# MariaPdg/thesis-fmri-reconstruction

Measured on NVIDIA B200. Metric: stage1_vaegan_train_samples_per_sec_64x64, higher is better.
Workload: dtype bf16

## Files before the change

thesis_fmri_reconstruction_b200/csrc/api.cu:

```cuda
#include <cstdarg>
#include <cstdio>
#include <cstring>
#include <cstdlib>
#include <algorithm>

#include "../../include/fmri_b200.h"
#include "simt_kernels.cuh"
#include "tc_kernels.cuh"
#include "hconv_kernels.cuh"
#include "hwgrad_kernels.cuh"
#include "cto3_kernels.cuh"
#include "mmd_kernels.cuh"
#include "eval_kernels.cuh"

using namespace fmri;

static thread_local char g_err[512] = "";
static int fail(int code, const char* fmt, ...) {
    va_list ap;
    va_start(ap, fmt);
    vsnprintf(g_err, sizeof(g_err), fmt, ap);
    va_end(ap);
    return code;
}
// ... 39 lines not shown
    }
    void* p = nullptr;
    return cudaMallocAsync(&p, bytes, st) == cudaSuccess ? p : nullptr;
}
#define SCRATCH(ptr, type, count, st)                                                                        \
    type* ptr = reinterpret_cast<type*>(scratch_alloc(sizeof(type) * (size_t)(count), st));                  \
    if (!ptr) return fail(FMRI_ERR_CUDA, "scratch allocation of %zu bytes", sizeof(type) * (size_t)(count))
template <typename T>
static int ordered_add(const T* part, int nparts, long long n, T* dst, cudaStream_t st) {
    ordered_add_kernel<T><<<grid1d(n, 256), 256, 0, st>>>(part, nparts, n, dst);
    LAUNCH_OK();
    return 0;
}

extern "C" int fmri_tensor_path_available(void) {
    int dev = 0, major = 0;
    if (cudaGetDevice(&dev) != cudaSuccess) {
        cudaGetLastError();
        return 0;
    }
    if (cudaDeviceGetAttribute(&major, cudaDevAttrComputeCapabilityMajor, dev) != cudaSuccess) {
        cudaGetLastError();
        return 0;
    }
    return major == 10 ? 1 : 0;
}

typedef CUresult (*EncodeTiledFn)(CUtensorMap*, CUtensorMapDataType, cuuint32_t, void*, const cuuint64_t*,
                                  const cuuint64_t*, const cuuint32_t*, const cuuint32_t*, CUtensorMapInterleave,
                                  CUtensorMapSwizzle, CUtensorMapL2promotion, CUtensorMapFloatOOBfill);
static EncodeTiledFn encode_fn() {
    static EncodeTiledFn fn = [] {
        void* p = nullptr;
        cudaDriverEntryPointQueryResult q;
        if (cudaGetDriverEntryPoint("cuTensorMapEncodeTiled", &p, cudaEnableDefault, &q) != cudaSuccess) p = nullptr;
        return reinterpret_cast<EncodeTiledFn>(p);
    }();
    return fn;
}
static int make_map(CUtensorMap* m, const void* base, int rank, const long long* dims, const long long* strides_el,
                    const int* box, int inner_bytes) {
    EncodeTiledFn fn = encode_fn();
    if (!fn) return fail(FMRI_ERR_CUDA, "cuTensorMapEncodeTiled entry point not found");
    cuuint64_t gd[4], gs[3];
    cuuint32_t bx[4], es[4];
    for (int i = 0; i < rank; ++i) {
        gd[i] = (cuuint64_t)dims[i];
        bx[i] = (cuuint32_t)box[i];
        es[i] = 1;
    }
    for (int i = 0; i + 1 < rank; ++i) gs[i] = (cuuint64_t)strides_el[i] * 2;
    const CUtensorMapSwizzle sw = inner_bytes == 128 ? CU_TENSOR_MAP_SWIZZLE_128B
                                 : inner_bytes == 64 ? CU_TENSOR_MAP_SWIZZLE_64B
                                                     : CU_TENSOR_MAP_SWIZZLE_32B;
    CUresult r = fn(m, CU_TENSOR_MAP_DATA_TYPE_BFLOAT16, (cuuint32_t)rank, const_cast<void*>(base), gd, gs, bx, es,
                    CU_TENSOR_MAP_INTERLEAVE_NONE, sw, CU_TENSOR_MAP_L2_PROMOTION_L2_256B,
                    CU_TENSOR_MAP_FLOAT_OOB_FILL_NONE);
    if (r != CUDA_SUCCESS)
        return fail(FMRI_ERR_CUDA,
                    "cuTensorMapEncodeTiled failed (%d): rank %d dims %lld %lld %lld %lld box %d %d %d %d stride0 %lld",
                    (int)r, rank, dims[0], dims[1], rank > 2 ? dims[2] : 0, rank > 3 ? dims[3] : 0, box[0], box[1],
                    rank > 2 ? box[2] : 0, rank > 3 ? box[3] : 0, strides_el[0]);
    return 0;
}
static int make_act_map(CUtensorMap* m, const void* base, int C, int X, int Y, int N, long long sx, long long sy,
                        long long sn, int box_c, int bw, int bh, int bn) {
    const long long dims[4] = {C, std::max(X, 1), std::max(Y, 1), N};
    const long long st[3] = {sx, sy, sn};
    const int box[4] = {box_c, bw, bh, bn};
    return make_map(m, base, 4, dims, st, box, box_c * 2);
}

template <int BN, int KCH, int STAGES, int MT>
static int launch_ig(const IgParams& p, int classes, cudaStream_t st) {
    using L = IgSmem<BN, KCH, STAGES, MT>;
    static bool attr_done = false;
    if (!attr_done) {
        CUDA_OK(cudaFuncSetAttribute(igemm_kernel<BN, KCH, STAGES, MT>, cudaFuncAttributeMaxDynamicSharedMemorySize,
                                     L::TOTAL));
        attr_done = true;
    }
    dim3 grid(cdiv((long long)p.tiles_x * p.tiles_y * p.tiles_n, MT), p.n_tiles * p.splits, classes);
    igemm_kernel<BN, KCH, STAGES, MT><<<grid, 192, L::TOTAL, st>>>(p);
    LAUNCH_OK();
    return 0;
}
template <int BN, int KCH, int STAGES, int MT, int EXTRA, bool YR = false>
static int launch_ig_persistent_x(const IgParams& p, int classes, cudaStream_t st) {
    using L = IgSmem<BN, KCH, STAGES, MT, YR, EXTRA, true>;
    static bool attr_done = false;
    if (!attr_done) {
        CUDA_OK(cudaFuncSetAttribute(igemm_persistent_kernel<BN, KCH, STAGES, MT, EXTRA, YR>,
                                     cudaFuncAttributeMaxDynamicSharedMemorySize, L::TOTAL));
        attr_done = true;
    }
    const long long m_groups = cdiv((long long)p.tiles_x * p.tiles_y * p.tiles_n, MT);
    const long long tiles = m_groups * p.n_tiles * classes;
    static int occ = 0;
    if (!occ) {
        CUDA_OK(cudaOccupancyMaxActiveBlocksPerMultiprocessor(&occ, igemm_persistent_kernel<BN, KCH, STAGES, MT, EXTRA, YR>,
                                                              IGP_THREADS, L::TOTAL));
        occ = std::max(1, occ);
    }
    const int per_sm = std::max(1, std::min<int>(std::min(2, 512 / (2 * MT * BN)), occ));
    const int grid = (int)std::min<long long>(tiles, 148LL * per_sm);
    igemm_persistent_kernel<BN, KCH, STAGES, MT, EXTRA, YR><<<grid, IGP_THREADS, L::TOTAL, st>>>(p, classes);
// ... 686 lines not shown
}

extern "C" int fmri_conv_wgrad(const fmri_conv_desc* d, const void* x, const void* dy, float* dw, int accumulate,
                               void* ws, size_t ws_bytes, void* stream) {
    int rc = check_conv(d);
    if (rc) return rc;
    int OH, OW;
    fmri_conv_out_hw(d, &OH, &OW);
    if (d->dtype == FMRI_BF16) {
        const size_t need = fmri_conv_wgrad_workspace(d);
        if (!ws || ws_bytes < need) return fail(FMRI_ERR_WORKSPACE, "conv wgrad workspace %zu < %zu", ws_bytes, need);
        if (d->stride != 2) return fail(FMRI_ERR_UNSUPPORTED, "stride-1 conv wgrad on the tensor path");
        CUDA_OK(cudaMemsetAsync(ws, 0, need, S(stream)));
        float* wsf = reinterpret_cast<float*>(ws);
        int Cd, Cs;
        if (!d->transposed) {
            Cd = d->Cout; Cs = d->Cin;
            rc = run_wgrad_tc(dy, d->N, OH, OW, Cd, x, d->H, d->W, Cs, 2, 25, wsf, S(stream));
        } else {
            Cd = d->Cin; Cs = d->Cout;
            rc = run_wgrad_tc(x, d->N, d->H, d->W, Cd, dy, OH, OW, Cs, 2, 25, wsf, S(stream));
        }
        if (rc) return rc;
        const long long n = 25LL * Cd * Cs;
        scatter4_kernel<float, float><<<grid1d(n, 256), 256, 0, S(stream)>>>(wsf, dw, 1, 25, Cd, Cs, 0, 1, 25LL * Cs,
                                                                            25, accumulate);
        LAUNCH_OK();
        return 0;
    }
    DirectWgradParams p;
    memset(&p, 0, sizeof(p));
    p.N = d->N;
    p.stride = d->stride;
    p.accumulate = accumulate;
    const float *A, *B;
    if (!d->transposed) {
        A = reinterpret_cast<const float*>(dy); p.PH = OH; p.PW = OW; p.Ca = d->Cout;
        B = reinterpret_cast<const float*>(x); p.BH = d->H; p.BW = d->W; p.Cb = d->Cin;
    } else {
        A = reinterpret_cast<const float*>(x); p.PH = d->H; p.PW = d->W; p.Ca = d->Cin;
        B = reinterpret_cast<const float*>(dy); p.BH = OH; p.BW = OW; p.Cb = d->Cout;
    }
    p.a_sn = (long long)p.PH * p.PW * p.Ca; p.a_sy = (long long)p.PW * p.Ca; p.a_sx = p.Ca; p.a_sc = 1;
    p.b_sn = (long long)p.BH * p.BW * p.Cb; p.b_sy = (long long)p.BW * p.Cb; p.b_sx = p.Cb; p.b_sc = 1;
    p.w_sa = 25LL * p.Cb;
    p.w_sb = 25;
    direct_wgrad_kernel<float, float><<<25 * p.Ca * p.Cb, 128, 0, S(stream)>>>(A, B, dw, p);
    LAUNCH_OK();
    return 0;
}

static const size_t HC_WS_PACK = 65536;
extern "C" size_t fmri_edge_workspace(const fmri_edge_desc* d) {
    return std::max(sizeof(float) * 75 * (size_t)d->C, HC_WS_PACK + (size_t)d->N * d->H * d->W * 16);
}

static bool hc_build(HcParams& p, HcPackSpec& spec, int N, int H, int W, int chunks, int stride, int OH, int OW, int BN,
                     bool flip) {
    memset(&p, 0, sizeof(p));
    memset(&spec, 0, sizeof(spec));
    p.N = N; p.H = H; p.W = W; p.chunks = chunks; p.OH = OH; p.OW = OW;
    const int hx = stride == 1 ? 4 : 2;
    if (stride == 1) {
        p.num_planes = 1;
        p.pl_ys[0] = p.pl_xs[0] = 1;
        p.pl_yoff[0] = p.pl_xoff[0] = -2;
    } else {
        p.num_planes = 4;
        for (int ph = 0; ph < 2; ++ph)
            for (int pw = 0; pw < 2; ++pw) {
                const int pl = ph * 2 + pw;
                p.pl_ys[pl] = p.pl_xs[pl] = 2;
                p.pl_yoff[pl] = ph - 2;
                p.pl_xoff[pl] = pw - 2;
            }
    }
    p.PW = OW + hx;
    if (p.PW > 200) return false;
    const int max_off = hx * p.PW + hx;
    const int nsteps = chunks >= 2 ? 25 * (chunks / 2) : 13;
    if (nsteps > HC_MAX_STEPS) return false;
    p.num_steps = nsteps;
    bool found = false;
    for (int pass = 0; pass < 2 && !found; ++pass) {
        const int mt_max = std::min(5, (pass == 0 ? 128 : 256) / BN);
        const size_t smem_cap = pass == 0 ? 110 * 1024 : 227 * 1024;
        double best = 0.0;
        for (int tht = std::min(OH, (mt_max * 128) / p.PW); tht >= 1; --tht) {
            HcParams q = p;
            q.THt = tht;
            q.tiles_y = cdiv(OH, tht);
            q.MT = cdiv((long long)tht * q.PW, 128);
            q.PH = tht + hx;
            q.slab_rows = (q.PH * q.PW + 7) / 8 * 8 + (chunks > 1 ? 2 : 0);
            const long long overshoot = ((long long)q.MT * 128 + max_off + 1 - q.slab_rows) * 16;
            if (overshoot > 0 && overshoot > hc_b_bytes(q, BN)) continue;
            if ((size_t)hc_smem_bytes(q, BN) > smem_cap) continue;
            const double eff = (double)OH * OW / ((double)q.tiles_y * q.MT * 128);
            if (eff > best + 1e-9) { best = eff; p = q; found = true; }
        }
    }
    if (!found) return false;
    int woff[25];
    for (int kh = 0; kh < 5; ++kh)
        for (int kw = 0; kw < 5; ++kw) {
            int plane = 0, dyr = kh, dxr = kw;
            if (stride == 2) {
// ... 101 lines not shown
    memset(&p, 0, sizeof(p));
    __nv_bfloat16* wt = reinterpret_cast<__nv_bfloat16*>(ws);
    c3_pack_weights_kernel<<<cdiv(C3_NB * C, 256), 256, 0, st>>>(w, wt, s_co, s_c, flip, C);
    LAUNCH_OK();
    if (make_act_map(&p.mapX, X, C, H * W, 1, N, C, (long long)H * W * C, (long long)H * W * C, C, 128, 1, 1)) return 1;
    {
        const long long dims[2] = {C, C3_NB};
        const long long stv[1] = {C};
        const int box[2] = {C, C3_NB};
        if (make_map(&p.mapW, wt, 2, dims, stv, box, C * 2)) return 1;
    }
    p.N = N; p.H = H; p.out = img; p.bias = bias; p.act = act;
    static bool attr_done = false;
    if (!attr_done) {
        CUDA_OK(cudaFuncSetAttribute(cto3_kernel, cudaFuncAttributeMaxDynamicSharedMemorySize, C3_SMEM));
        attr_done = true;
    }
    cto3_kernel<<<std::min(N, 148), C3_THREADS, C3_SMEM, st>>>(p);
    LAUNCH_OK();
    return 0;
}

static int hconv_c_to_3(const void* X, int N, int H, int W, int C, const float* w, long long s_co, long long s_c, int flip,
                        const float* bias, int act, float* img, void* ws, cudaStream_t st) {
    if (C != 32 && C != 64) return 1;
    {
        const int rc = cto3_run(X, N, H, W, C, w, s_co, s_c, flip, bias, act, img, ws, st);
        if (rc <= 0) return rc;
    }
    HcParams p;
    HcPackSpec spec;
    if (!hc_build(p, spec, N, H, W, C / 8, 1, H, W, 16, flip != 0)) return 1;
    p.X = reinterpret_cast<const __nv_bfloat16*>(X);
    p.epi = 0; p.out = img; p.bias = bias; p.act = act; p.n_out = 3;
    return hc_run(p, spec, 16, w, 3, C, s_co, s_c, ws, st);
}

static int hconv_3_to_c(const float* i0, const float* i1, const float* i2, int nps, int N, int H, int W, int C, int stride,
                        const float* w, long long s_c, long long s_ci, int flip, const float* bias, int act, void* y,
                        void* ws, cudaStream_t st) {
    if (C != 32 && C != 64) return 1;
    const int OH = (H - 1) / stride + 1, OW = (W - 1) / stride + 1;
    HcParams p;
    HcPackSpec spec;
    if (!hc_build(p, spec, N, H, W, 1, stride, OH, OW, C, flip != 0)) return 1;
    __nv_bfloat16* img8 = reinterpret_cast<__nv_bfloat16*>(reinterpret_cast<uint8_t*>(ws) + HC_WS_PACK);
    img8_pack_kernel<<<grid1d((long long)N * H * W, 256), 256, 0, st>>>(i0, i1, i2, nps, N, (long long)H * W, img8);
    LAUNCH_OK();
    p.X = img8;
    p.epi = 1; p.out = y; p.bias = bias; p.act = act; p.n_out = C;
    return hc_run(p, spec, C, w, C, 3, s_c, s_ci, ws, st);
}

static int g_hw_variant = -1;
static int hwgrad_run(const void* T, const float* i0, const float* i1, const float* i2, int nps, int N, int PH, int PW, int C,
                      float* dwk, float* dbias, int flip, void* ws, cudaStream_t st, int plane = -1, int IH = 0, int IW = 0) {
    if (g_hw_variant < 0) {
        const char* e = getenv("FMRI_HWGRAD");
        g_hw_variant = e ? atoi(e) : 0;
    }
    if (g_hw_variant == 2) return 1;
    if (C != 32 && C != 64) return 1;
    HwParams p;
    memset(&p, 0, sizeof(p));
    p.N = N; p.PH = PH; p.PW = PW; p.C = C;
    p.PWp = (PW + 4 + 15) / 16 * 16;
    if (p.PWp > 128) return 1;
    static int bh_cap = 0;
    if (!bh_cap) {
        const char* e = getenv("FMRI_HW_BH");
        bh_cap = e ? std::max(1, atoi(e)) : 2;
    }
    p.bh = std::max(1, std::min(std::min(PH, bh_cap), 256 / p.PWp));
    p.tiles_y = cdiv(PH, p.bh);
    p.slab_rows = ((p.bh + 4) * p.PWp + 16 + 7) / 8 * 8;
    p.d_chunk = (p.bh * p.PWp * 128 + 1023) / 1024 * 1024;
    p.stages = 2;
    if (hw_smem_bytes(p) > 227 * 1024) return 1;
    while (p.stages < HW_MAX_STAGES) {
        ++p.stages;
        if (hw_smem_bytes(p) > 110 * 1024) { --p.stages; break; }
    }
    const long long dims[4] = {C, PW, PH, N};
    const long long strides[3] = {C, (long long)PW * C, (long long)PH * PW * C};
    const int box[4] = {64, p.PWp, p.bh, 1};
    if (make_map(&p.mapT, T, 4, dims, strides, box, 128)) return 1;
    __nv_bfloat16* img8 = reinterpret_cast<__nv_bfloat16*>(reinterpret_cast<uint8_t*>(ws) + HC_WS_PACK);
    p.kh0 = 0; p.nkh = 5;
    if (plane < 0) {
        img8_pack_kernel<<<grid1d((long long)N * PH * PW, 256), 256, 0, st>>>(i0, i1, i2, nps, N, (long long)PH * PW, img8);
    } else {
        p.plane = 1; p.ph = plane >> 1; p.pw = plane & 1;
        p.kh0 = 1; p.nkh = p.ph ? 2 : 3;
        img8_plane_pack_kernel<<<grid1d((long long)N * PH * PW, 256), 256, 0, st>>>(i0, i1, i2, nps, N, IH, IW, PH, PW, p.ph,
                                                                                   p.pw, img8);
    }
    LAUNCH_OK();
    p.img8 = img8;
    p.dwk = dwk; p.dbias = dbias; p.flip = flip; p.desc_variant = g_hw_variant;
    const int smem = hw_smem_bytes(p);
    static int attr_smem = 0;
    if (smem > attr_smem) {
        CUDA_OK(cudaFuncSetAttribute(hwgrad_kernel, cudaFuncAttributeMaxDynamicSharedMemorySize, smem));
        attr_smem = smem;
    }
    const int total = N * p.tiles_y;
    const int nb = std::min(total, 148 * (smem <= 110 * 1024 ? 2 : 1));
    const long long nw = 75LL * C;
    SCRATCH(part, float, (long long)nb * (nw + C), st);
    CUDA_OK(cudaMemsetAsync(part, 0, sizeof(float) * (size_t)nb * (nw + C), st));
    p.dwk = part;
    p.dbias = dbias ? part + nb * nw : nullptr;
    hwgrad_kernel<<<nb, HW_THREADS, smem, st>>>(p);
    LAUNCH_OK();
    int rc = ordered_add(part, nb, nw, dwk, st);
    if (!rc && dbias) rc = ordered_add(part + nb * nw, nb, C, dbias, st);
    CUDA_OK(cudaFreeAsync(part, st));
    return rc;
}

static int check_edge(const fmri_edge_desc* d, const void* ws, size_t ws_bytes) {
    if (!d || (d->C != 32 && d->C != 64)) return fail(FMRI_ERR_UNSUPPORTED, "edge conv supports C in {32,64}");
    if (d->stride != 1 && d->stride != 2) return fail(FMRI_ERR_ARG, "edge stride");
    if (!ws || ws_bytes < fmri_edge_workspace(d)) return fail(FMRI_ERR_WORKSPACE, "edge workspace too small");
    return 0;
}
static int pack_edge_in(const fmri_edge_desc* d, const float* w, float* wk, cudaStream_t st) {
    permute4_kernel<float, float><<<grid1d(75LL * d->C, 256), 256, 0, st>>>(w, wk, 1, 3, 25, d->C, 0, 25, 1, 75, 0);
    LAUNCH_OK();
    return 0;
}
static int pack_edge_out(const fmri_edge_desc* d, const float* w, float* wk, int flip, cudaStream_t st) {
    permute4_kernel<float, float><<<grid1d(75LL * d->C, 256), 256, 0, st>>>(
        flip ? w + 24 : w, wk, 1, 3, 25, d->C, 0, 25LL * d->C, flip ? -1 : 1, 25, 0);
    LAUNCH_OK();
    return 0;
}
template <int C>
static int edge_in_fprop_t(const fmri_edge_desc* d, const float* i0, const float* i1, const float* i2, int nps,
                           const float* wk, const float* bias, int act, void* y, int OH, int OW, cudaStream_t st) {
    const long long pix = (long long)d->N * OH * OW;
    if (d->dtype == FMRI_BF16)
        edge3_to_c_kernel<C, __nv_bfloat16><<<cdiv(pix, 128), 128, 0, st>>>(
            i0, i1, i2, nps, wk, bias, reinterpret_cast<__nv_bfloat16*>(y), d->N, d->H, d->W, OH, OW, d->stride, act);
    else
        edge3_to_c_kernel<C, float><<<cdiv(pix, 128), 128, 0, st>>>(i0, i1, i2, nps, wk, bias,
                                                                   reinterpret_cast<float*>(y), d->N, d->H, d->W, OH,
                                                                   OW, d->stride, act);
    LAUNCH_OK();
    return 0;
}
extern "C" int fmri_edge_in_fprop(const fmri_edge_desc* d, const float* img0, const float* img1, const float* img2,
                                  int n_per_src, const float* w, const float* bias, int act, void* y, void* ws,
                                  size_t ws_bytes, void* stream) {
    int rc = check_edge(d, ws, ws_bytes);
    if (rc) return rc;
    if (!img1) img1 = img0;
    if (!img2) img2 = img0;
    if (d->dtype == FMRI_BF16 && fmri_tensor_path_available()) {
        rc = hconv_3_to_c(img0, img1, img2, n_per_src, d->N, d->H, d->W, d->C, d->stride, w, 75, 25, 0, bias, act, y, ws,
                          S(stream));
        if (rc <= 0) return rc;
    }
    float* wk = reinterpret_cast<float*>(ws);
    rc = pack_edge_in(d, w, wk, S(stream));
    if (rc) return rc;
    const int OH = (d->H - 1) / d->stride + 1, OW = (d->W - 1) / d->stride + 1;
// ... 24 lines not shown
    }
    float* wk = reinterpret_cast<float*>(ws);
    rc = pack_edge_in(d, w, wk, S(stream));
    if (rc) return rc;
    const int flip = d->stride == 1 ? 1 : 0;
    return d->C == 32 ? edge_to3_t<32>(d->dtype, dy, wk, nullptr, dimg, d->N, OH, OW, d->H, d->W, d->stride, flip, 0,
                                       S(stream))
                      : edge_to3_t<64>(d->dtype, dy, wk, nullptr, dimg, d->N, OH, OW, d->H, d->W, d->stride, flip, 0,
                                       S(stream));
}
template <int C>
static int edge_wgrad_t(int dtype, const void* T, const float* i0, const float* i1, const float* i2, int nps,
                        float* dwk, float* dbias, int N, int PH, int PW, int IH, int IW, int stride, int sg,
                        cudaStream_t st) {
    if (PW <= 128 && (PW - 1) * stride + 5 <= 144) {
        const long long lines = (long long)N * PH;
        const int rpb = (int)std::max<long long>(1, (lines + 148 * 3 - 1) / (148 * 3));
        const int blocks = cdiv(lines, rpb);
        if (dtype == FMRI_BF16)
            edge_wgrad_rows_kernel<C, __nv_bfloat16><<<blocks, 256, 0, st>>>(
                reinterpret_cast<const __nv_bfloat16*>(T), i0, i1, i2, nps, dwk, dbias, N, PH, PW, IH, IW, stride, sg, rpb);
        else
            edge_wgrad_rows_kernel<C, float><<<blocks, 256, 0, st>>>(reinterpret_cast<const float*>(T), i0, i1, i2, nps,
                                                                    dwk, dbias, N, PH, PW, IH, IW, stride, sg, rpb);
        LAUNCH_OK();
        return 0;
    }
    if (dbias) return fail(FMRI_ERR_UNSUPPORTED, "edge wgrad: fused bias gradient needs rows of <= 128 pixels");
    const long long pix = (long long)N * PH * PW;
    int ppb = (int)std::max<long long>(64, ((pix + 148 * 4 - 1) / (148 * 4) + 7) / 8 * 8);
    const int blocks = cdiv(pix, ppb);
    if (dtype == FMRI_BF16)
        edge_wgrad_kernel<C, __nv_bfloat16><<<blocks, 256, 0, st>>>(reinterpret_cast<const __nv_bfloat16*>(T), i0, i1,
                                                                    i2, nps, dwk, N, PH, PW, IH, IW, stride, sg, ppb);
    else
        edge_wgrad_kernel<C, float><<<blocks, 256, 0, st>>>(reinterpret_cast<const float*>(T), i0, i1, i2, nps, dwk, N,
                                                            PH, PW, IH, IW, stride, sg, ppb);
    LAUNCH_OK();
    return 0;
}
extern "C" int fmri_edge_in_wgrad(const fmri_edge_desc* d, const float* img0, const float* img1, const float* img2,
                                  int n_per_src, const void* dy, float* dw, float* dbias, int accumulate, void* ws,
                                  size_t ws_bytes, void* stream) {
    int rc = check_edge(d, ws, ws_bytes);
    if (rc) return rc;
    float* dwk = reinterpret_cast<float*>(ws);
    CUDA_OK(cudaMemsetAsync(dwk, 0, sizeof(float) * 75 * (size_t)d->C, S(stream)));
    const int OH = (d->H - 1) / d->stride + 1, OW = (d->W - 1) / d->stride + 1;
    if (!img1) img1 = img0;
    if (!img2) img2 = img0;
    if (dbias && !accumulate) CUDA_OK(cudaMemsetAsync(dbias, 0, sizeof(float) * d->C, S(stream)));
    rc = 1;
    if (d->dtype == FMRI_BF16 && d->stride == 1 && fmri_tensor_path_available())
        rc = hwgrad_run(dy, img0, img1, img2, n_per_src, d->N, d->H, d->W, d->C, dwk, dbias, 0, ws, S(stream));
    else if (d->dtype == FMRI_BF16 && d->stride == 2 && !dbias && fmri_tensor_path_available()) {
        for (int plane = 0; plane < 4; ++plane) {
            rc = hwgrad_run(dy, img0, img1, img2, n_per_src, d->N, OH, OW, d->C, dwk, nullptr, 0, ws, S(stream), plane, d->H, d->W);
            if (rc) break;
        }
        if (rc == 1) CUDA_OK(cudaMemsetAsync(dwk, 0, sizeof(float) * 75 * (size_t)d->C, S(stream)));
    }
    if (rc == 1)
        rc = d->C == 32 ? edge_wgrad_t<32>(d->dtype, dy, img0, img1, img2, n_per_src, dwk, dbias, d->N, OH, OW, d->H, d->W,
                                           d->stride, 1, S(stream))
                        : edge_wgrad_t<64>(d->dtype, dy, img0, img1, img2, n_per_src, dwk, dbias, d->N, OH, OW, d->H, d->W,
                                           d->stride, 1, S(stream));
    if (rc) return rc;
    scatter4_kernel<float, float><<<grid1d(75LL * d->C, 256), 256, 0, S(stream)>>>(dwk, dw, 1, 3, 25, d->C, 0, 25, 1,
                                                                                  75, accumulate);
    LAUNCH_OK();
    return 0;
}
extern "C" int fmri_edge_out_fprop(const fmri_edge_desc* d, const void* x, const float* w, const float* bias, int act,
                                   float* img, void* ws, size_t ws_bytes, void* stream) {
    int rc = check_edge(d, ws, ws_bytes);
    if (rc) return rc;
    if (d->stride != 1) return fail(FMRI_ERR_UNSUPPORTED, "edge out conv is stride 1");
    if (d->dtype == FMRI_BF16 && fmri_tensor_path_available()) {
        rc = hconv_c_to_3(x, d->N, d->H, d->W, d->C, w, 25LL * d->C, 25, 0, bias, act, img, ws, S(stream));
        if (rc <= 0) return rc;
    }
    float* wk = reinterpret_cast<float*>(ws);
    rc = pack_edge_out(d, w, wk, 0, S(stream));
    if (rc) return rc;
    return d->C == 32
               ? edge_to3_t<32>(d->dtype, x, wk, bias, img, d->N, d->H, d->W, d->H, d->W, 1, 0, act, S(stream))
               : edge_to3_t<64>(d->dtype, x, wk, bias, img, d->N, d->H, d->W, d->H, d->W, 1, 0, act, S(stream));
}
extern "C" int fmri_edge_out_dgrad(const fmri_edge_desc* d, const float* dimg, const float* w, void* dx, void* ws,
                                   size_t ws_bytes, void* stream) {
    int rc = check_edge(d, ws, ws_bytes);
    if (rc) return rc;
    if (d->stride != 1) return fail(FMRI_ERR_UNSUPPORTED, "edge out conv is stride 1");
    if (d->dtype == FMRI_BF16 && fmri_tensor_path_available()) {
        rc = hconv_3_to_c(dimg, dimg, dimg, d->N, d->N, d->H, d->W, d->C, 1, w, 25, 25LL * d->C, 1, nullptr, 0, dx, ws,
                          S(stream));
        if (rc <= 0) return rc;
    }
    float* wk = reinterpret_cast<float*>(ws);
    rc = pack_edge_out(d, w, wk, 1, S(stream));
    if (rc) return rc;
    fmri_edge_desc e = *d;
    return e.C == 32 ? edge_in_fprop_t<32>(&e, dimg, dimg, dimg, d->N, wk, nullptr, 0, dx, d->H, d->W, S(stream))
                     : edge_in_fprop_t<64>(&e, dimg, dimg, dimg, d->N, wk, nullptr, 0, dx, d->H, d->W, S(stream));
}
extern "C" int fmri_edge_out_wgrad(const fmri_edge_desc* d, const void* x, const float* dimg, float* dw,
                                   int accumulate, void* ws, size_t ws_bytes, void* stream) {
    int rc = check_edge(d, ws, ws_bytes);
    if (rc) return rc;
    if (d->stride != 1) return fail(FMRI_ERR_UNSUPPORTED, "edge out conv is stride 1");
    float* dwk = reinterpret_cast<float*>(ws);
    CUDA_OK(cudaMemsetAsync(dwk, 0, sizeof(float) * 75 * (size_t)d->C, S(stream)));
    rc = 1;
    if (d->dtype == FMRI_BF16 && fmri_tensor_path_available())
        rc = hwgrad_run(x, dimg, dimg, dimg, d->N, d->N, d->H, d->W, d->C, dwk, nullptr, 1, ws, S(stream));
    if (rc == 1)
        rc = d->C == 32 ? edge_wgrad_t<32>(d->dtype, x, dimg, dimg, dimg, d->N, dwk, nullptr, d->N, d->H, d->W, d->H, d->W,
                                           1, -1, S(stream))
                        : edge_wgrad_t<64>(d->dtype, x, dimg, dimg, dimg, d->N, dwk, nullptr, d->N, d->H, d->W, d->H, d->W,
                                           1, -1, S(stream));
    if (rc) return rc;
    scatter4_kernel<float, float><<<grid1d(75LL * d->C, 256), 256, 0, S(stream)>>>(dwk, dw, 1, 3, 25, d->C, 0,
                                                                                  25LL * d->C, 1, 25, accumulate);
    LAUNCH_OK();
    return 0;
}

static int transpose_any(const void* src, int sdt, void* dst, int ddt, int N, int R, int Cc, int accumulate, cudaStream_t st);
extern "C" int fmri_linear_pack_weights(const fmri_linear_desc* d, const float* w, void* wp, int ldw, void* wpt,
                                        int ldwt, void* stream) {
    if (!d || d->M < 0 || d->N <= 0 || d->K <= 0) return fail(FMRI_ERR_ARG, "bad linear descriptor");
    if (wp) {
        if (ldw < d->K) return fail(FMRI_ERR_ARG, "ldw < K");
        int rc = fmri_cast2d(w, FMRI_F32, d->K, wp, FMRI_BF16, ldw, d->N, d->K, stream);
        if (rc) return rc;
    }
    if (wpt) {
        if (ldwt < d->N) return fail(FMRI_ERR_ARG, "ldwt < N");
        if (ldwt == d->N) {
            int rc = transpose_any(w, FMRI_F32, wpt, FMRI_BF16, 1, d->N, d->K, 0, S(stream));
            if (rc) return rc;
        } else {
            scatter4_kernel<float, __nv_bfloat16><<<grid1d((long long)d->N * d->K, 256), 256, 0, S(stream)>>>(
                w, reinterpret_cast<__nv_bfloat16*>(wpt), 1, 1, d->N, d->K, 0, 0, 1, ldwt, 0);
            LAUNCH_OK();
        }
    }
    return 0;
}

template <typename Ta, typename Tb, typename Tc>
static int simt_gemm(const Ta* A, long long a_sm, long long a_sk, const Tb* B, long long b_sn, long long b_sk, Tc* C,
                     long long c_sm, long long c_sn, const float* bias, int M, int N, int K, int act, int accumulate,
                     cudaStream_t st) {
    dim3 grid(cdiv(N, 64), cdiv(M, 64));
    simt_gemm_kernel<Ta, Tb, Tc><<<grid, 256, 0, st>>>(A, a_sm, a_sk, B, b_sn, b_sk, C, c_sm, c_sn, bias, M, N, K,
                                                      act, accumulate);
    LAUNCH_OK();
    return 0;
}

extern "C" int fmri_linear_fprop(const fmri_linear_desc* d, const void* x, int ldx, const float* w, const void* wp,
                                 int ldw, const float* bias, int act, void* y, int ldy, int y_dtype, void* stream) {
    if (!d || d->M <= 0 || d->N <= 0 || d->K <= 0) return fail(FMRI_ERR_ARG, "bad linear descriptor");
    if (d->dtype == FMRI_BF16) {
        if (!wp) return fail(FMRI_ERR_ARG, "bf16 linear needs packed weights");
        if (d->N % 32 == 0)
            return run_gemm_tn(x, ldx, wp, ldw, d->M, d->N, d->K, bias, act, y, ldy, y_dtype == FMRI_F32, 0, S(stream));
// ... 655 lines not shown
```

thesis_fmri_reconstruction_b200/csrc/hconv_kernels.cuh:

```cuda
#pragma once
#include "ptx.cuh"

namespace fmri {

struct HcStep {
    uint32_t a_off;
    uint32_t a_lbo;
    uint32_t b_off;
};
constexpr int HC_MAX_STEPS = 104;

struct HcParams {
    const __nv_bfloat16* X;
    int N, H, W;
    int chunks;
    int num_planes;
    int pl_ys[4], pl_xs[4];
    int pl_yoff[4], pl_xoff[4];
    int PW, PH;
    int issuers_max;
    int slab_rows;
    int num_steps;
    HcStep steps[HC_MAX_STEPS];
    int THt, tiles_y;
// ... 222 lines not shown
                        if (valid) {
                            *reinterpret_cast<uint4*>(o + c0) = make_uint4(pk[0], pk[1], pk[2], pk[3]);
                            *reinterpret_cast<uint4*>(o + c0 + 8) = make_uint4(pk[4], pk[5], pk[6], pk[7]);
                        }
                    }
                }
            }
            tc_fence_before();
            __syncwarp();
            if (lane == 0) mbar_arrive(&tmem_empty[sb]);
        }
    }
    tc_fence_before();
    __syncthreads();
    tc_fence_after();
    if (warp == 0) tmem_dealloc(tmem_base, tmem_cols);
}

struct HcPackSpec {
    int16_t tap[HC_MAX_STEPS][2];
    int16_t cb[HC_MAX_STEPS][2];
};
__global__ void hc_pack_weights_kernel(const float* __restrict__ w, __nv_bfloat16* __restrict__ dst,
                                       const __grid_constant__ HcPackSpec spec, int num_steps, int BN, int n_real,
                                       int c_real, long long s_n, long long s_c) {
    const int rows = num_steps * BN;
    const int total = 2 * rows * 8;
    for (int i = blockIdx.x * blockDim.x + threadIdx.x; i < total; i += gridDim.x * blockDim.x) {
        const int e = i & 7;
        const int rr = (i >> 3) % rows;
        const int h = (i >> 3) / rows;
        const int s = rr / BN, n = rr - s * BN;
        const int tap = spec.tap[s][h], c = spec.cb[s][h] + e;
        float v = 0.f;
        if (tap >= 0 && n < n_real && c < c_real) v = __ldg(w + n * s_n + c * s_c + tap);
        dst[i] = __float2bfloat16_rn(v);
    }
}

__global__ void img8_pack_kernel(const float* __restrict__ s0, const float* __restrict__ s1, const float* __restrict__ s2,
                                 int n_per_src, int N, long long HW, __nv_bfloat16* __restrict__ dst) {
    const long long total = (long long)N * HW;
    for (long long i = blockIdx.x * (long long)blockDim.x + threadIdx.x; i < total; i += (long long)gridDim.x * blockDim.x) {
        const int n = (int)(i / HW);
        const long long px = i - (long long)n * HW;
        const int si = n / n_per_src;
        const float* img = (si == 0 ? s0 : (si == 1 ? s1 : s2)) + (long long)(n - si * n_per_src) * 3 * HW + px;
        const uint32_t a = pack_bf16x2(__ldg(img), __ldg(img + HW));
        const uint32_t b = pack_bf16x2(__ldg(img + 2 * HW), 0.f);
        *reinterpret_cast<uint4*>(dst + i * 8) = make_uint4(a, b, 0u, 0u);
    }
}

__global__ void img8_plane_pack_kernel(const float* __restrict__ s0, const float* __restrict__ s1, const float* __restrict__ s2,
                                       int n_per_src, int N, int IH, int IW, int PH, int PW, int ph, int pw,
                                       __nv_bfloat16* __restrict__ dst) {
    const long long total = (long long)N * PH * PW;
    for (long long i = blockIdx.x * (long long)blockDim.x + threadIdx.x; i < total; i += (long long)gridDim.x * blockDim.x) {
        const int x = (int)(i % PW);
        const int y = (int)((i / PW) % PH);
        const int n = (int)(i / ((long long)PW * PH));
        const int iy = 2 * y + ph, ix = 2 * x + pw;
        uint32_t a = 0u, b = 0u;
        if (iy < IH && ix < IW) {
            const int si = n / n_per_src;
            const float* img = (si == 0 ? s0 : (si == 1 ? s1 : s2)) + (long long)(n - si * n_per_src) * 3 * IH * IW +
                               (long long)iy * IW + ix;
            const long long HW = (long long)IH * IW;
            a = pack_bf16x2(__ldg(img), __ldg(img + HW));
            b = pack_bf16x2(__ldg(img + 2 * HW), 0.f);
        }
        *reinterpret_cast<uint4*>(dst + i * 8) = make_uint4(a, b, 0u, 0u);
    }
}

}
```

thesis_fmri_reconstruction_b200/csrc/hwgrad_kernels.cuh:

```cuda
#pragma once
#include "ptx.cuh"
#include "hconv_kernels.cuh"

namespace fmri {

struct HwParams {
    CUtensorMap mapT;
    const __nv_bfloat16* img8;
    int N, PH, PW, C;
    int PWp, bh;
    int tiles_y;
    int slab_rows;
    float* dwk;
    float* dbias;
    int flip;
    int desc_variant;
    int stages;
    int d_chunk;
    int kh0, nkh;
    int plane;
    int ph, pw;
};

constexpr int HW_MAX_STAGES = 8;
constexpr int HW_THREADS = 384;
constexpr int HW_PRODUCERS = 160;
__host__ __device__ inline int hw_stage_bytes(const HwParams& p) { return 2 * p.d_chunk + ((p.slab_rows * 16 + 1023) / 1024) * 1024; }
__host__ __device__ inline int hw_smem_bytes(const HwParams& p) { return p.stages * hw_stage_bytes(p) + 4096 + 256 + 1024; }

__global__ void __launch_bounds__(HW_THREADS) hwgrad_kernel(const __grid_constant__ HwParams p) {
    extern __shared__ uint8_t smem_raw[];
    uint8_t* smem = reinterpret_cast<uint8_t*>((reinterpret_cast<uintptr_t>(smem_raw) + 1023) & ~uintptr_t(1023));
    const int stage_bytes = hw_stage_bytes(p);
    const int HW_STAGES = p.stages;
    uint8_t* s_ones = smem + HW_STAGES * stage_bytes;
    uint64_t* bars = reinterpret_cast<uint64_t*>(s_ones + 4096);
    uint64_t* full_bar = bars;
    uint64_t* empty_bar = bars + HW_MAX_STAGES;
    uint64_t* tmem_full = bars + 2 * HW_MAX_STAGES;
    uint32_t* tmem_slot = reinterpret_cast<uint32_t*>(bars + 2 * HW_MAX_STAGES + 1);

    const int warp = threadIdx.x >> 5, lane = threadIdx.x & 31;
    const int total_tiles = p.N * p.tiles_y;
    const int rows = p.bh * p.PWp;
    constexpr uint32_t TMEM_COLS = 256;
    const int n_issuers = p.nkh + (p.dbias ? 1 : 0);

    if (threadIdx.x == 0) {
        tma_prefetch_desc(&p.mapT);
        for (int s = 0; s < HW_STAGES; ++s) {
            mbar_init(&full_bar[s], 1 + HW_PRODUCERS);
            mbar_init(&empty_bar[s], n_issuers);
        }
        mbar_init(tmem_full, n_issuers);
        fence_barrier_init();
    }
    if (warp == 1) tmem_alloc(tmem_slot, TMEM_COLS);
    for (int i = threadIdx.x; i < 4096 / 4; i += HW_THREADS) reinterpret_cast<uint32_t*>(s_ones)[i] = 0x3F803F80u;
    for (int s = 0; s < HW_STAGES; ++s) {
        uint32_t* st = reinterpret_cast<uint32_t*>(smem + s * stage_bytes);
        for (int i = threadIdx.x; i < stage_bytes / 4; i += HW_THREADS) st[i] = 0u;
    }
    fence_proxy_async_smem();
    tc_fence_before();
    __syncthreads();
    tc_fence_after();
    const uint32_t tmem_base = *tmem_slot;

    if (warp == 0) {
        if (lane == 0) {
            int it = 0;
            for (int t = blockIdx.x; t < total_tiles; t += gridDim.x, ++it) {
                const int st = it % HW_STAGES;
                const uint32_t ph = (it / HW_STAGES) & 1;
                const int n = t / p.tiles_y, y0 = (t - n * p.tiles_y) * p.bh;
                mbar_wait(&empty_bar[st], ph ^ 1);
                mbar_arrive_expect_tx(&full_bar[st], rows * 128);
                tma_load_4d(smem + st * stage_bytes, &p.mapT, &full_bar[st], 0, 0, y0, n);
            }
        }
        __syncwarp();
    }
    const int issuer = warp == 1 ? 0 : (warp == 7 ? 1 : (warp >= 8 ? warp - 6 : -1));
    if (issuer >= 0 && issuer < n_issuers) {
        const uint32_t idesc = umma_idesc_bf16(64, 48, true, true);
        const uint32_t idesc1 = umma_idesc_bf16(64, 16, true, true);
        const uint32_t tmem_u = __shfl_sync(0xffffffffu, tmem_base, 0);
        const uint32_t b_lbo = p.desc_variant ? 16 : 128, b_sbo = p.desc_variant ? 128 : 16;
        const int ksteps = rows / 16;
        int it = 0;
        for (int t = blockIdx.x; t < total_tiles; t += gridDim.x, ++it) {
            const int st = it % HW_STAGES;
            const uint32_t ph = (it / HW_STAGES) & 1;
            mbar_wait(&full_bar[st], ph);
            tc_fence_after();
            const uint32_t sd = smem_u32(smem + st * stage_bytes);
            const uint32_t ss = sd + 2 * p.d_chunk;
            const uint64_t adesc = umma_smem_desc(sd, p.d_chunk, 8 * 128, UMMA_SW128);
            if (issuer < p.nkh) {
                const int kh = p.kh0 + issuer;
                const uint64_t bdesc = umma_smem_desc(ss, b_lbo, b_sbo, 0) + (uint32_t)(kh * p.PWp);
                for (int k = 0; k < ksteps; ++k)
                    umma_bf16_elect(tmem_u + kh * 48, adesc + ((k * 16 * 128) >> 4), bdesc + (uint32_t)(k * 16), idesc,
                                    (it | k) != 0);
            } else {
                const uint64_t odesc = umma_smem_desc(smem_u32(s_ones), b_lbo, b_sbo, 0);
                for (int k = 0; k < ksteps; ++k)
                    umma_bf16_elect(tmem_u + 240, adesc + ((k * 16 * 128) >> 4), odesc + (uint32_t)(k * 16), idesc1, (it | k) != 0);
            }
            umma_commit_elect(&empty_bar[st]);
        }
        umma_commit_elect(tmem_full);
        __syncwarp();
    }
    if (warp == 0 || warp == 1 || warp == 7) {
    } else if (warp >= 2 && warp < 2 + HW_PRODUCERS / 32) {
        const int ptid = threadIdx.x - 64;
        const int halo_px = (p.bh + 4) * p.PWp;
        int it = 0;
        for (int t = blockIdx.x; t < total_tiles; t += gridDim.x, ++it) {
            const int st = it % HW_STAGES;
            const uint32_t ph = (it / HW_STAGES) & 1;
            const int n = t / p.tiles_y, y0 = (t - n * p.tiles_y) * p.bh;
            mbar_wait(&empty_bar[st], ph ^ 1);
            const uint32_t ss = smem_u32(smem + st * stage_bytes) + 2 * p.d_chunk;
            const __nv_bfloat16* In = p.img8 + (size_t)n * p.PH * p.PW * 8;
            int row = ptid;
            int sy = row / p.PWp, sx = row - sy * p.PWp;
            for (; row < halo_px; row += HW_PRODUCERS) {
                const int iy = y0 + sy - 2, ix = sx - 2;
                const bool ok = iy >= 0 && iy < p.PH && ix >= 0 && ix < p.PW;
                cp_async16(ss + row * 16, ok ? In + ((size_t)iy * p.PW + ix) * 8 : In, ok ? 16u : 0u);
                sx += HW_PRODUCERS;
                while (sx >= p.PWp) { sx -= p.PWp; ++sy; }
            }
            cp_async_wait_all();
            fence_proxy_async_smem();
            mbar_arrive(&full_bar[st]);
        }
    }
    if (warp >= 8) {
        mbar_wait(tmem_full, 0);
        tc_fence_after();
        const int q = warp & 3;
        const int c = q * 16 + lane;
        const bool valid = lane < 16 && c < p.C;
        for (int kh = p.kh0; kh < p.kh0 + p.nkh; ++kh) {
#pragma unroll 1
            for (int part = 0; part < 3; ++part) {
                uint32_t v[16];
                tmem_ld16(tmem_base + (static_cast<uint32_t>(q * 32) << 16) + kh * 48 + part * 16, v);
                tmem_ld_wait();
                if (!valid) continue;
#pragma unroll
                for (int h = 0; h < 2; ++h) {
                    const int kw = part * 2 + h;
                    if (kw >= 5) continue;
                    int tap = kh * 5 + kw;
                    if (p.plane) {
                        const int rkh = 2 * (kh - 1) + p.ph, rkw = 2 * (kw - 1) + p.pw;
                        if (kh < 1 || kw < 1 || rkh > 4 || rkw > 4) continue;
                        tap = rkh * 5 + rkw;
                    }
                    if (p.flip) tap = 24 - tap;
#pragma unroll
                    for (int ci = 0; ci < 3; ++ci)
                        atomicAdd(p.dwk + (size_t)blockIdx.x * 75 * p.C + (size_t)(ci * 25 + tap) * p.C + c,
                                  __uint_as_float(v[h * 8 + ci]));
                }
            }
        }
        if (p.dbias) {
            uint32_t v[16];
            tmem_ld16(tmem_base + (static_cast<uint32_t>(q * 32) << 16) + 240, v);
            tmem_ld_wait();
            if (valid) atomicAdd(p.dbias + (size_t)blockIdx.x * p.C + c, __uint_as_float(v[0]));
        }
        tc_fence_before();
    }
    __syncthreads();
    tc_fence_after();
    if (warp == 1) tmem_dealloc(tmem_base, TMEM_COLS);
}

}
```

Before: 39280.

## Load hwgrad image halo via TMA with packed pair layout and window-split MMAs

Replaces the cp.async producer warps that gathered image pixels in the weight-gradient kernel with a second TMA load from a new pre-padded pack layout. The layout holds two adjacent pixels plus a constant one per 16-byte row, so the bias gradient comes out of the same MMA and the separate ones-matrix pass is dropped. MMAs are now split by horizontal window instead of by kernel row. The stride-2 plane loop moves inside the run function, reusing one tensor map and one partial buffer, and per-block atomics become plain stores. The cost is a more intricate descriptor and column mapping, plus a larger pack workspace.

```diff
diff --git a/thesis_fmri_reconstruction_b200/csrc/api.cu b/thesis_fmri_reconstruction_b200/csrc/api.cu
--- a/thesis_fmri_reconstruction_b200/csrc/api.cu
+++ b/thesis_fmri_reconstruction_b200/csrc/api.cu
@@ -115,6 +115,7 @@
     for (int i = 0; i + 1 < rank; ++i) gs[i] = (cuuint64_t)strides_el[i] * 2;
     const CUtensorMapSwizzle sw = inner_bytes == 128 ? CU_TENSOR_MAP_SWIZZLE_128B
                                  : inner_bytes == 64 ? CU_TENSOR_MAP_SWIZZLE_64B
+                                 : inner_bytes == 0  ? CU_TENSOR_MAP_SWIZZLE_NONE
                                                      : CU_TENSOR_MAP_SWIZZLE_32B;
     CUresult r = fn(m, CU_TENSOR_MAP_DATA_TYPE_BFLOAT16, (cuuint32_t)rank, const_cast<void*>(base), gd, gs, bx, es,
                     CU_TENSOR_MAP_INTERLEAVE_NONE, sw, CU_TENSOR_MAP_L2_PROMOTION_L2_256B,
@@ -907,7 +908,8 @@
 
 static const size_t HC_WS_PACK = 65536;
 extern "C" size_t fmri_edge_workspace(const fmri_edge_desc* d) {
-    return std::max(sizeof(float) * 75 * (size_t)d->C, HC_WS_PACK + (size_t)d->N * d->H * d->W * 16);
+    const size_t row = (size_t)(d->W + 4 + 15) / 16 * 16;
+    return std::max(sizeof(float) * 75 * (size_t)d->C, HC_WS_PACK + (size_t)d->N * d->H * row * 16);
 }
 
 static bool hc_build(HcParams& p, HcPackSpec& spec, int N, int H, int W, int chunks, int stride, int OH, int OW, int BN,
@@ -1115,52 +1117,38 @@
     return hc_run(p, spec, C, w, C, 3, s_c, s_ci, ws, st);
 }
 
-static int g_hw_variant = -1;
 static int hwgrad_run(const void* T, const float* i0, const float* i1, const float* i2, int nps, int N, int PH, int PW, int C,
-                      float* dwk, float* dbias, int flip, void* ws, cudaStream_t st, int plane = -1, int IH = 0, int IW = 0) {
-    if (g_hw_variant < 0) {
-        const char* e = getenv("FMRI_HWGRAD");
-        g_hw_variant = e ? atoi(e) : 0;
-    }
-    if (g_hw_variant == 2) return 1;
+                      float* dwk, float* dbias, int flip, void* ws, cudaStream_t st, int stride, int IH, int IW) {
     if (C != 32 && C != 64) return 1;
     HwParams p;
     memset(&p, 0, sizeof(p));
     p.N = N; p.PH = PH; p.PW = PW; p.C = C;
     p.PWp = (PW + 4 + 15) / 16 * 16;
     if (p.PWp > 128) return 1;
-    static int bh_cap = 0;
-    if (!bh_cap) {
-        const char* e = getenv("FMRI_HW_BH");
-        bh_cap = e ? std::max(1, atoi(e)) : 2;
-    }
-    p.bh = std::max(1, std::min(std::min(PH, bh_cap), 256 / p.PWp));
+    p.bh = std::max(1, std::min(std::min(PH, 2), 256 / p.PWp));
     p.tiles_y = cdiv(PH, p.bh);
-    p.slab_rows = ((p.bh + 4) * p.PWp + 16 + 7) / 8 * 8;
-    p.d_chunk = (p.bh * p.PWp * 128 + 1023) / 1024 * 1024;
+    p.a_bytes = p.bh * p.PWp * 128;
+    p.b_bytes = (((p.bh + 4) * p.PWp + 16) * 16 + 1023) / 1024 * 1024;
     p.stages = 2;
     if (hw_smem_bytes(p) > 227 * 1024) return 1;
     while (p.stages < HW_MAX_STAGES) {
         ++p.stages;
         if (hw_smem_bytes(p) > 110 * 1024) { --p.stages; break; }
     }
-    const long long dims[4] = {C, PW, PH, N};
-    const long long strides[3] = {C, (long long)PW * C, (long long)PH * PW * C};
-    const int box[4] = {64, p.PWp, p.bh, 1};
-    if (make_map(&p.mapT, T, 4, dims, strides, box, 128)) return 1;
-    __nv_bfloat16* img8 = reinterpret_cast<__nv_bfloat16*>(reinterpret_cast<uint8_t*>(ws) + HC_WS_PACK);
-    p.kh0 = 0; p.nkh = 5;
-    if (plane < 0) {
-        img8_pack_kernel<<<grid1d((long long)N * PH * PW, 256), 256, 0, st>>>(i0, i1, i2, nps, N, (long long)PH * PW, img8);
-    } else {
-        p.plane = 1; p.ph = plane >> 1; p.pw = plane & 1;
-        p.kh0 = 1; p.nkh = p.ph ? 2 : 3;
-        img8_plane_pack_kernel<<<grid1d((long long)N * PH * PW, 256), 256, 0, st>>>(i0, i1, i2, nps, N, IH, IW, PH, PW, p.ph,
-                                                                                   p.pw, img8);
-    }
-    LAUNCH_OK();
-    p.img8 = img8;
-    p.dwk = dwk; p.dbias = dbias; p.flip = flip; p.desc_variant = g_hw_variant;
+    {
+        const long long dims[4] = {C, PW, PH, N};
+        const long long strides[3] = {C, (long long)PW * C, (long long)PH * PW * C};
+        const int box[4] = {64, p.PWp, p.bh, 1};
+        if (make_map(&p.mapT, T, 4, dims, strides, box, 128)) return 1;
+    }
+    __nv_bfloat16* pack = reinterpret_cast<__nv_bfloat16*>(reinterpret_cast<uint8_t*>(ws) + HC_WS_PACK);
+    {
+        const long long dims[4] = {128, p.PWp / 16, PH, N};
+        const long long strides[3] = {128, (long long)p.PWp * 8, (long long)PH * p.PWp * 8};
+        const int box[4] = {128, p.PWp / 16, p.bh + 4, 1};
+        if (make_map(&p.mapX, pack, 4, dims, strides, box, 0)) return 1;
+    }
+    p.flip = flip;
     const int smem = hw_smem_bytes(p);
     static int attr_smem = 0;
     if (smem > attr_smem) {
@@ -1174,8 +1162,19 @@
     CUDA_OK(cudaMemsetAsync(part, 0, sizeof(float) * (size_t)nb * (nw + C), st));
     p.dwk = part;
     p.dbias = dbias ? part + nb * nw : nullptr;
-    hwgrad_kernel<<<nb, HW_THREADS, smem, st>>>(p);
-    LAUNCH_OK();
+    const dim3 pack_block(p.PWp, 256 / p.PWp);
+    const int pack_grid = (int)std::min<long long>(cdiv((long long)N * PH, pack_block.y), 148 * 16);
+    for (int plane = 0; plane < (stride == 2 ? 4 : 1); ++plane) {
+        p.kh0 = 0; p.nkh = 5;
+        if (stride == 2) {
+            p.plane = 1; p.ph = plane >> 1; p.pw = plane & 1;
+            p.kh0 = 1; p.nkh = p.ph ? 2 : 3;
+        }
+        hw_pack_kernel<<<pack_grid, pack_block, 0, st>>>(i0, i1, i2, nps, N, IH, IW, PH, PW, p.PWp, stride, p.ph, p.pw, pack);
+        LAUNCH_OK();
+        hwgrad_kernel<<<nb, HW_THREADS, smem, st>>>(p);
+        LAUNCH_OK();
+    }
     int rc = ordered_add(part, nb, nw, dwk, st);
     if (!rc && dbias) rc = ordered_add(part + nb * nw, nb, C, dbias, st);
     CUDA_OK(cudaFreeAsync(part, st));
@@ -1306,14 +1305,9 @@
     if (dbias && !accumulate) CUDA_OK(cudaMemsetAsync(dbias, 0, sizeof(float) * d->C, S(stream)));
     rc = 1;
     if (d->dtype == FMRI_BF16 && d->stride == 1 && fmri_tensor_path_available())
-        rc = hwgrad_run(dy, img0, img1, img2, n_per_src, d->N, d->H, d->W, d->C, dwk, dbias, 0, ws, S(stream));
-    else if (d->dtype == FMRI_BF16 && d->stride == 2 && !dbias && fmri_tensor_path_available()) {
-        for (int plane = 0; plane < 4; ++plane) {
-            rc = hwgrad_run(dy, img0, img1, img2, n_per_src, d->N, OH, OW, d->C, dwk, nullptr, 0, ws, S(stream), plane, d->H, d->W);
-            if (rc) break;
-        }
-        if (rc == 1) CUDA_OK(cudaMemsetAsync(dwk, 0, sizeof(float) * 75 * (size_t)d->C, S(stream)));
-    }
+        rc = hwgrad_run(dy, img0, img1, img2, n_per_src, d->N, d->H, d->W, d->C, dwk, dbias, 0, ws, S(stream), 1, d->H, d->W);
+    else if (d->dtype == FMRI_BF16 && d->stride == 2 && !dbias && fmri_tensor_path_available())
+        rc = hwgrad_run(dy, img0, img1, img2, n_per_src, d->N, OH, OW, d->C, dwk, nullptr, 0, ws, S(stream), 2, d->H, d->W);
     if (rc == 1)
         rc = d->C == 32 ? edge_wgrad_t<32>(d->dtype, dy, img0, img1, img2, n_per_src, dwk, dbias, d->N, OH, OW, d->H, d->W,
                                            d->stride, 1, S(stream))
@@ -1367,7 +1361,7 @@
     CUDA_OK(cudaMemsetAsync(dwk, 0, sizeof(float) * 75 * (size_t)d->C, S(stream)));
     rc = 1;
     if (d->dtype == FMRI_BF16 && fmri_tensor_path_available())
-        rc = hwgrad_run(x, dimg, dimg, dimg, d->N, d->N, d->H, d->W, d->C, dwk, nullptr, 1, ws, S(stream));
+        rc = hwgrad_run(x, dimg, dimg, dimg, d->N, d->N, d->H, d->W, d->C, dwk, nullptr, 1, ws, S(stream), 1, d->H, d->W);
     if (rc == 1)
         rc = d->C == 32 ? edge_wgrad_t<32>(d->dtype, x, dimg, dimg, dimg, d->N, dwk, nullptr, d->N, d->H, d->W, d->H, d->W,
                                            1, -1, S(stream))
diff --git a/thesis_fmri_reconstruction_b200/csrc/hconv_kernels.cuh b/thesis_fmri_reconstruction_b200/csrc/hconv_kernels.cuh
--- a/thesis_fmri_reconstruction_b200/csrc/hconv_kernels.cuh
+++ b/thesis_fmri_reconstruction_b200/csrc/hconv_kernels.cuh
@@ -298,26 +298,4 @@
     }
 }
 
-__global__ void img8_plane_pack_kernel(const float* __restrict__ s0, const float* __restrict__ s1, const float* __restrict__ s2,
-                                       int n_per_src, int N, int IH, int IW, int PH, int PW, int ph, int pw,
-                                       __nv_bfloat16* __restrict__ dst) {
-    const long long total = (long long)N * PH * PW;
-    for (long long i = blockIdx.x * (long long)blockDim.x + threadIdx.x; i < total; i += (long long)gridDim.x * blockDim.x) {
-        const int x = (int)(i % PW);
-        const int y = (int)((i / PW) % PH);
-        const int n = (int)(i / ((long long)PW * PH));
-        const int iy = 2 * y + ph, ix = 2 * x + pw;
-        uint32_t a = 0u, b = 0u;
-        if (iy < IH && ix < IW) {
-            const int si = n / n_per_src;
-            const float* img = (si == 0 ? s0 : (si == 1 ? s1 : s2)) + (long long)(n - si * n_per_src) * 3 * IH * IW +
-                               (long long)iy * IW + ix;
-            const long long HW = (long long)IH * IW;
-            a = pack_bf16x2(__ldg(img), __ldg(img + HW));
-            b = pack_bf16x2(__ldg(img + 2 * HW), 0.f);
-        }
-        *reinterpret_cast<uint4*>(dst + i * 8) = make_uint4(a, b, 0u, 0u);
-    }
-}
-
-}
+}
diff --git a/thesis_fmri_reconstruction_b200/csrc/hwgrad_kernels.cuh b/thesis_fmri_reconstruction_b200/csrc/hwgrad_kernels.cuh
--- a/thesis_fmri_reconstruction_b200/csrc/hwgrad_kernels.cuh
+++ b/thesis_fmri_reconstruction_b200/csrc/hwgrad_kernels.cuh
@@ -6,17 +6,15 @@
 
 struct HwParams {
     CUtensorMap mapT;
-    const __nv_bfloat16* img8;
+    CUtensorMap mapX;
     int N, PH, PW, C;
     int PWp, bh;
     int tiles_y;
-    int slab_rows;
+    int a_bytes, b_bytes;
+    int stages;
     float* dwk;
     float* dbias;
     int flip;
-    int desc_variant;
-    int stages;
-    int d_chunk;
     int kh0, nkh;
     int plane;
     int ph, pw;
@@ -24,17 +22,41 @@
 
 constexpr int HW_MAX_STAGES = 8;
 constexpr int HW_THREADS = 384;
-constexpr int HW_PRODUCERS = 160;
-__host__ __device__ inline int hw_stage_bytes(const HwParams& p) { return 2 * p.d_chunk + ((p.slab_rows * 16 + 1023) / 1024) * 1024; }
-__host__ __device__ inline int hw_smem_bytes(const HwParams& p) { return p.stages * hw_stage_bytes(p) + 4096 + 256 + 1024; }
+__host__ __device__ inline int hw_smem_bytes(const HwParams& p) { return p.stages * (p.a_bytes + p.b_bytes) + 256 + 1024; }
+
+__global__ void hw_pack_kernel(const float* __restrict__ s0, const float* __restrict__ s1, const float* __restrict__ s2,
+                               int n_per_src, int N, int IH, int IW, int PH, int PW, int PWp, int s, int ph, int pw,
+                               __nv_bfloat16* __restrict__ dst) {
+    const int xx = threadIdx.x;
+    const long long HW = (long long)IH * IW;
+    for (int r = blockIdx.x * blockDim.y + threadIdx.y; r < N * PH; r += gridDim.x * blockDim.y) {
+        const int n = r / PH, y = r - n * PH;
+        const int iy = s * y + ph;
+        float v[6] = {0.f, 0.f, 0.f, 0.f, 0.f, 0.f};
+        if (iy < IH) {
+            const int si = n / n_per_src;
+            const float* img = (si == 0 ? s0 : (si == 1 ? s1 : s2)) + (long long)(n - si * n_per_src) * 3 * HW + (long long)iy * IW;
+#pragma unroll
+            for (int h = 0; h < 2; ++h) {
+                const int x = xx - 2 + h, ix = s * x + pw;
+                if (x >= 0 && x < PW && ix < IW) {
+                    v[3 * h] = __ldg(img + ix);
+                    v[3 * h + 1] = __ldg(img + HW + ix);
+                    v[3 * h + 2] = __ldg(img + 2 * HW + ix);
+                }
+            }
+        }
+        *reinterpret_cast<uint4*>(dst + ((long long)r * PWp + xx) * 8) =
+            make_uint4(pack_bf16x2(v[0], v[1]), pack_bf16x2(v[2], v[3]), pack_bf16x2(v[4], v[5]), pack_bf16x2(1.f, 0.f));
+    }
+}
 
 __global__ void __launch_bounds__(HW_THREADS) hwgrad_kernel(const __grid_constant__ HwParams p) {
     extern __shared__ uint8_t smem_raw[];
     uint8_t* smem = reinterpret_cast<uint8_t*>((reinterpret_cast<uintptr_t>(smem_raw) + 1023) & ~uintptr_t(1023));
-    const int stage_bytes = hw_stage_bytes(p);
+    const int stage_bytes = p.a_bytes + p.b_bytes;
     const int HW_STAGES = p.stages;
-    uint8_t* s_ones = smem + HW_STAGES * stage_bytes;
-    uint64_t* bars = reinterpret_cast<uint64_t*>(s_ones + 4096);
+    uint64_t* bars = reinterpret_cast<uint64_t*>(smem + HW_STAGES * stage_bytes);
     uint64_t* full_bar = bars;
     uint64_t* empty_bar = bars + HW_MAX_STAGES;
     uint64_t* tmem_full = bars + 2 * HW_MAX_STAGES;
@@ -43,20 +65,20 @@
     const int warp = threadIdx.x >> 5, lane = threadIdx.x & 31;
     const int total_tiles = p.N * p.tiles_y;
     const int rows = p.bh * p.PWp;
+    const int nwin = p.plane ? 2 : 3;
     constexpr uint32_t TMEM_COLS = 256;
-    const int n_issuers = p.nkh + (p.dbias ? 1 : 0);
 
     if (threadIdx.x == 0) {
         tma_prefetch_desc(&p.mapT);
+        tma_prefetch_desc(&p.mapX);
         for (int s = 0; s < HW_STAGES; ++s) {
-            mbar_init(&full_bar[s], 1 + HW_PRODUCERS);
-            mbar_init(&empty_bar[s], n_issuers);
+            mbar_init(&full_bar[s], 1);
+            mbar_init(&empty_bar[s], nwin);
         }
-        mbar_init(tmem_full, n_issuers);
+        mbar_init(tmem_full, nwin);
         fence_barrier_init();
     }
     if (warp == 1) tmem_alloc(tmem_slot, TMEM_COLS);
-    for (int i = threadIdx.x; i < 4096 / 4; i += HW_THREADS) reinterpret_cast<uint32_t*>(s_ones)[i] = 0x3F803F80u;
     for (int s = 0; s < HW_STAGES; ++s) {
         uint32_t* st = reinterpret_cast<uint32_t*>(smem + s * stage_bytes);
         for (int i = threadIdx.x; i < stage_bytes / 4; i += HW_THREADS) st[i] = 0u;
@@ -69,93 +91,60 @@
 
     if (warp == 0) {
         if (lane == 0) {
+            const uint32_t tx = rows * 128 + (p.bh + 4) * p.PWp * 16;
             int it = 0;
             for (int t = blockIdx.x; t < total_tiles; t += gridDim.x, ++it) {
                 const int st = it % HW_STAGES;
                 const uint32_t ph = (it / HW_STAGES) & 1;
                 const int n = t / p.tiles_y, y0 = (t - n * p.tiles_y) * p.bh;
                 mbar_wait(&empty_bar[st], ph ^ 1);
-                mbar_arrive_expect_tx(&full_bar[st], rows * 128);
-                tma_load_4d(smem + st * stage_bytes, &p.mapT, &full_bar[st], 0, 0, y0, n);
+                mbar_arrive_expect_tx(&full_bar[st], tx);
+                uint8_t* sa = smem + st * stage_bytes;
+                tma_load_4d(sa, &p.mapT, &full_bar[st], 0, 0, y0, n);
+                tma_load_4d(sa + p.a_bytes, &p.mapX, &full_bar[st], 0, 0, y0 - 2, n);
             }
         }
         __syncwarp();
-    }
-    const int issuer = warp == 1 ? 0 : (warp == 7 ? 1 : (warp >= 8 ? warp - 6 : -1));
-    if (issuer >= 0 && issuer < n_issuers) {
-        const uint32_t idesc = umma_idesc_bf16(64, 48, true, true);
-        const uint32_t idesc1 = umma_idesc_bf16(64, 16, true, true);
+    } else if (warp >= 1 && warp <= nwin) {
+        const int win = warp - 1;
+        const uint32_t idesc = umma_idesc_bf16(64, 8 * p.nkh, true, true);
         const uint32_t tmem_u = __shfl_sync(0xffffffffu, tmem_base, 0);
-        const uint32_t b_lbo = p.desc_variant ? 16 : 128, b_sbo = p.desc_variant ? 128 : 16;
-        const int ksteps = rows / 16;
         int it = 0;
         for (int t = blockIdx.x; t < total_tiles; t += gridDim.x, ++it) {
             const int st = it % HW_STAGES;
             const uint32_t ph = (it / HW_STAGES) & 1;
             mbar_wait(&full_bar[st], ph);
             tc_fence_after();
-            const uint32_t sd = smem_u32(smem + st * stage_bytes);
-            const uint32_t ss = sd + 2 * p.d_chunk;
-            const uint64_t adesc = umma_smem_desc(sd, p.d_chunk, 8 * 128, UMMA_SW128);
-            if (issuer < p.nkh) {
-                const int kh = p.kh0 + issuer;
-                const uint64_t bdesc = umma_smem_desc(ss, b_lbo, b_sbo, 0) + (uint32_t)(kh * p.PWp);
-                for (int k = 0; k < ksteps; ++k)
-                    umma_bf16_elect(tmem_u + kh * 48, adesc + ((k * 16 * 128) >> 4), bdesc + (uint32_t)(k * 16), idesc,
-                                    (it | k) != 0);
-            } else {
-                const uint64_t odesc = umma_smem_desc(smem_u32(s_ones), b_lbo, b_sbo, 0);
-                for (int k = 0; k < ksteps; ++k)
-                    umma_bf16_elect(tmem_u + 240, adesc + ((k * 16 * 128) >> 4), odesc + (uint32_t)(k * 16), idesc1, (it | k) != 0);
-            }
+            const uint32_t sa = smem_u32(smem + st * stage_bytes);
+            const uint64_t adesc = umma_smem_desc(sa, 8 * 128, 8 * 128, UMMA_SW128);
+            const uint64_t bdesc = umma_smem_desc(sa + p.a_bytes, 128, p.PWp * 16, 0) + (uint32_t)(p.kh0 * p.PWp + 2 * win);
+            const int ksteps = rows / 16;
+            for (int k = 0; k < ksteps; ++k)
+                umma_bf16_elect(tmem_u + win * 64, adesc + ((k * 16 * 128) >> 4), bdesc + (uint32_t)(k * 16), idesc,
+                                (it | k) != 0);
             umma_commit_elect(&empty_bar[st]);
         }
         umma_commit_elect(tmem_full);
         __syncwarp();
-    }
-    if (warp == 0 || warp == 1 || warp == 7) {
-    } else if (warp >= 2 && warp < 2 + HW_PRODUCERS / 32) {
-        const int ptid = threadIdx.x - 64;
-        const int halo_px = (p.bh + 4) * p.PWp;
-        int it = 0;
-        for (int t = blockIdx.x; t < total_tiles; t += gridDim.x, ++it) {
-            const int st = it % HW_STAGES;
-            const uint32_t ph = (it / HW_STAGES) & 1;
-            const int n = t / p.tiles_y, y0 = (t - n * p.tiles_y) * p.bh;
-            mbar_wait(&empty_bar[st], ph ^ 1);
-            const uint32_t ss = smem_u32(smem + st * stage_bytes) + 2 * p.d_chunk;
-            const __nv_bfloat16* In = p.img8 + (size_t)n * p.PH * p.PW * 8;
-            int row = ptid;
-            int sy = row / p.PWp, sx = row - sy * p.PWp;
-            for (; row < halo_px; row += HW_PRODUCERS) {
-                const int iy = y0 + sy - 2, ix = sx - 2;
-                const bool ok = iy >= 0 && iy < p.PH && ix >= 0 && ix < p.PW;
-                cp_async16(ss + row * 16, ok ? In + ((size_t)iy * p.PW + ix) * 8 : In, ok ? 16u : 0u);
-                sx += HW_PRODUCERS;
-                while (sx >= p.PWp) { sx -= p.PWp; ++sy; }
-            }
-            cp_async_wait_all();
-            fence_proxy_async_smem();
-            mbar_arrive(&full_bar[st]);
-        }
-    }
-    if (warp >= 8) {
+    } else if (warp >= 8) {
         mbar_wait(tmem_full, 0);
         tc_fence_after();
         const int q = warp & 3;
         const int c = q * 16 + lane;
-        const bool valid = lane < 16 && c < p.C;
-        for (int kh = p.kh0; kh < p.kh0 + p.nkh; ++kh) {
-#pragma unroll 1
-            for (int part = 0; part < 3; ++part) {
-                uint32_t v[16];
-                tmem_ld16(tmem_base + (static_cast<uint32_t>(q * 32) << 16) + kh * 48 + part * 16, v);
-                tmem_ld_wait();
-                if (!valid) continue;
+        float* dw = p.dwk + (size_t)blockIdx.x * 75 * p.C;
+        for (int win = 0; win < nwin; ++win) {
+            uint32_t v[32], u[16];
+            const uint32_t tad = tmem_base + (static_cast<uint32_t>(q * 32) << 16) + win * 64;
+            tmem_ld32(tad, v);
+            tmem_ld16(tad + 32, u);
+            tmem_ld_wait();
+            if (lane >= 16 || c >= p.C) continue;
+#pragma unroll
+            for (int j = 0; j < 5; ++j)
 #pragma unroll
                 for (int h = 0; h < 2; ++h) {
-                    const int kw = part * 2 + h;
-                    if (kw >= 5) continue;
+                    const int kh = p.kh0 + j, kw = 2 * win + h;
+                    if (j >= p.nkh || kw >= 5) continue;
                     int tap = kh * 5 + kw;
                     if (p.plane) {
                         const int rkh = 2 * (kh - 1) + p.ph, rkw = 2 * (kw - 1) + p.pw;
@@ -164,17 +153,12 @@
                     }
                     if (p.flip) tap = 24 - tap;
 #pragma unroll
-                    for (int ci = 0; ci < 3; ++ci)
-                        atomicAdd(p.dwk + (size_t)blockIdx.x * 75 * p.C + (size_t)(ci * 25 + tap) * p.C + c,
-                                  __uint_as_float(v[h * 8 + ci]));
+                    for (int ci = 0; ci < 3; ++ci) {
+                        const int col = j * 8 + h * 3 + ci;
+                        dw[(ci * 25 + tap) * p.C + c] = __uint_as_float(col < 32 ? v[col] : u[col - 32]);
+                    }
                 }
-            }
-        }
-        if (p.dbias) {
-            uint32_t v[16];
-            tmem_ld16(tmem_base + (static_cast<uint32_t>(q * 32) << 16) + 240, v);
-            tmem_ld_wait();
-            if (valid) atomicAdd(p.dbias + (size_t)blockIdx.x * p.C + c, __uint_as_float(v[0]));
+            if (p.dbias && win == 1) p.dbias[(size_t)blockIdx.x * p.C + c] = __uint_as_float(v[2 * 8 + 6]);
         }
         tc_fence_before();
     }
```

Measured after the change: 40240 (median of 6 runs). +2.4%, better.
